# SunJiamei/LRP-ImageCaptioning

Measured on AMD Instinct MI355X. Metric: LRP heatmaps/sec (per predicted token) VGG16+adaptive-attn, 224x224, higher is better.
Workload: dtype bf16x3; 1 GPU; batch=32 synthetic 224x224 per GPU, VGG16 + adaptive-attention, LRP per-token heat-maps, 10 words/caption, V=10000 (BASELINE configs[1]); parallelism=image-sharded x1, RCCL weight broadcast, reverse_walk_precision=bf16x3, handles_per_gpu=2

## Files before the change

### lrp-imagecaptioning_amd/csrc/common.h

```cpp
#pragma once
#include <hip/hip_runtime.h>
#include <atomic>
#include <cstdarg>
#include <cstdio>
#include <cstdlib>
#include <string>
#include <vector>

#include "../../include/lrp_hip.h"

namespace lrp {

inline std::atomic<unsigned long long> g_launch_count{0};
#undef hipLaunchKernelGGL
#define hipLaunchKernelGGL(kernelName, numBlocks, numThreads, memPerBlock, streamId, ...)                  \
  do {                                                                                                    \
    ::lrp::g_launch_count.fetch_add(1, std::memory_order_relaxed);                                       \
    kernelName<<<(numBlocks), (numThreads), (memPerBlock), (streamId)>>>(__VA_ARGS__);                   \
  } while (0)

std::string& last_error_ref();

struct Switches {
  int conv_halo = 1;
  int conv_breg = 1;
  int conv_breg8 = 1;
  int conv_breg4 = 1;
  int conv_small = 1;
  int conv_mid = 1;
  int epi_fast = 1;
  int up2_pw = 1;
  int tile_order = 1;
  int fwd_emit = 1;
  int fwd_il = 1;
  int img_fused = 1;
  int up2_compact = 1;
  int img_fold = 1;
  int pool_fused = 1;
  int sparse_pool = 1;
  void load() {
    *this = Switches();
    auto rd = [](const char* name, int& v) { if (const char* e = getenv(name)) v = atoi(e); };
    rd("LRP_CONV_HALO", conv_halo); rd("LRP_CONV_BREG", conv_breg); rd("LRP_CONV_SMALL", conv_small);
    rd("LRP_CONV_MID", conv_mid); rd("LRP_EPI_FAST", epi_fast); rd("LRP_UP2_PW", up2_pw); rd("LRP_TILE_ORDER", tile_order);
    rd("LRP_FWD_EMIT", fwd_emit); rd("LRP_FWD_IL", fwd_il); rd("LRP_IMG_FUSED", img_fused); rd("LRP_UP2_COMPACT", up2_compact);
    rd("LRP_IMG_FOLD", img_fold); rd("LRP_SPARSE_POOL", sparse_pool); rd("LRP_POOL_FUSED", pool_fused);
    if (const char* e = getenv("LRP_CONV_BREG8")) conv_breg8 = atoi(e);
    if (const char* e = getenv("LRP_CONV_BREG4")) conv_breg4 = atoi(e);
  }
};
inline Switches& sw() {
  static Switches s = [] { Switches t; t.load(); return t; }();
  return s;
}

inline int fail(int code, const char* fmt, ...) {
  char buf[512];
  va_list ap;
  va_start(ap, fmt);
  vsnprintf(buf, sizeof(buf), fmt, ap);
  va_end(ap);
  last_error_ref() = buf;
  return code;
}

#define LRP_HIP_CHECK(expr)                                                                     \
  do {                                                                                          \
    hipError_t _e = (expr);                                                                     \
    if (_e != hipSuccess)                                                                       \
      return ::lrp::fail(LRP_ERR_HIP, "%s failed: %s (%s:%d)", #expr, hipGetErrorString(_e), \
                         __FILE__, __LINE__);                                                   \
  } while (0)

#define LRP_TRY(expr)         \
  do {                        \
    int _rc = (expr);         \
    if (_rc != LRP_OK) return _rc; \
  } while (0)

struct DevBuf {
  void* p = nullptr;
  size_t bytes = 0;
  bool owned = true;
  DevBuf() = default;
  DevBuf(const DevBuf&) = delete;
  DevBuf& operator=(const DevBuf&) = delete;
  DevBuf(DevBuf&& o) noexcept : p(o.p), bytes(o.bytes), owned(o.owned) { o.p = nullptr; o.bytes = 0; o.owned = true; }
  DevBuf& operator=(DevBuf&& o) noexcept {
    if (this != &o) { release(); p = o.p; bytes = o.bytes; owned = o.owned; o.p = nullptr; o.bytes = 0; o.owned = true; }
    return *this;
  }
  ~DevBuf() { release(); }
  void release() {
    if (p && owned) (void)hipFree(p);
    p = nullptr;
    bytes = 0;
    owned = true;
  }
  void view_of(const DevBuf& arena, size_t offset, size_t n) {
    release();
    p = static_cast<char*>(arena.p) + offset;
    bytes = n;
    owned = false;
  }
  int alloc(size_t n, int64_t* total) {
    release();
    if (n == 0) n = 16;
    hipError_t e = hipMalloc(&p, n);
    if (e != hipSuccess) {
      p = nullptr;
      (void)hipGetLastError();
      return fail(LRP_ERR_NOMEM, "device memory: hipMalloc(%zu bytes) failed: %s", n, hipGetErrorString(e));
    }
    bytes = n;
    if (total) *total += (int64_t)n;
    return LRP_OK;
  }
  template <typename T>
  T* as() const { return reinterpret_cast<T*>(p); }
};

struct ProfileRec {
  hipEvent_t e0, e1;
  double flop;
};
struct Profiler {
  bool on = false;
  ProfileRec cur{};
  std::vector<ProfileRec> recs;
  void begin(hipStream_t st) {
    if (on) { (void)hipEventCreate(&cur.e0); (void)hipEventCreate(&cur.e1); (void)hipEventRecord(cur.e0, st); }
  }
  void end(hipStream_t st, double flop) {
    if (on) { (void)hipEventRecord(cur.e1, st); cur.flop = flop; recs.push_back(cur); }
  }
  template <typename F>
  void drain(F each) {
    for (ProfileRec& p : recs) {
      float t = 0.f;
      if (hipEventSynchronize(p.e1) == hipSuccess && hipEventElapsedTime(&t, p.e0, p.e1) == hipSuccess) each((double)t, p.flop);
      (void)hipEventDestroy(p.e0); (void)hipEventDestroy(p.e1);
    }
    recs.clear();
  }
  int records(int cap, double* ms_out, double* flop_out, int* n_out) {
    int k = 0;
    drain([&](double ms, double flop) { if (k < cap) { ms_out[k] = ms; flop_out[k] = flop; ++k; } });
    *n_out = k;
    return LRP_OK;
  }
  int query(int64_t* launches, double* ms, double* flop) {
    int64_t nl = 0; double tm = 0, fl = 0;
    drain([&](double t, double f) { tm += t; fl += f; ++nl; });
    if (launches) *launches = nl;
    if (ms) *ms = tm;
    if (flop) *flop = fl;
    return LRP_OK;
  }
};

}
```

### lrp-imagecaptioning_amd/csrc/conv_sparse.h

```cpp
#pragma once
#include "cnn_kernels.h"
#include "conv_igemm.h"

namespace lrp {

typedef __bf16 bf16x16 __attribute__((ext_vector_type(16)));
typedef unsigned u32x2 __attribute__((ext_vector_type(2)));

struct SparseArgs {
  const float* sc;
  const unsigned* idxp;
  const float* wsp;
  const float* gate;
  float* out;
  const int* row2img;
  int NB, Hp, Wp, C, N;
  int cols_t, m_tiles, n_tiles;
  int out_plain;
  int diag;
};

constexpr int SP_TW = 14, SP_PITCH = SP_TW + 2;
constexpr int SP_BPACK = 32768, SP_NSTAGE = 4;

template <int WMW_, int WNW_, int MI_, int NJ_, int TH_>
struct SparseTile {
  static constexpr int WMW = WMW_, WNW = WNW_, MI = MI_, NJ = NJ_, TH = TH_;
  static constexpr int NW = WMW * WNW, NT = 64 * NW;
  static constexpr int BM = WMW * MI * 32, BN = WNW * NJ * 32;
  static constexpr int NENT = (TH + 2) * SP_PITCH;
  static constexpr int PENT = NENT + 1;
  static constexpr int SUB = PENT * 16;
  static constexpr int ABUF = 3 * SUB;
  static constexpr int SUBPIECES = (PENT + 63) / 64;
  static constexpr int APIECES = 3 * SUBPIECES;
  static constexpr int ASLOTS = (APIECES + NW - 1) / NW;
  static constexpr int PLANE = BN * 16;
  static constexpr int BSTAGE = 8 * PLANE;
  static constexpr int BPIECES = BSTAGE / 1024 / NW;
  static constexpr int NSLAB = BM / 64;
  static constexpr int EPI_P = 64 * (BN / 8) / NT;
  static constexpr int LDS = SP_NSTAGE * BSTAGE + 2 * ABUF + 128;
  static_assert(TH * SP_TW <= BM && BM % 64 == 0 && 256 % BN == 0, "tile");
  static_assert(BPIECES * NW * 1024 == BSTAGE && EPI_P * NT == 64 * (BN / 8), "pieces");
  static_assert(SP_NSTAGE * BSTAGE >= 64 * BN * 4, "the epilogue's C slab lies in the B stages");
  static_assert((TH + 2) * 4 <= 128, "image table");
  static_assert(LDS <= 160 * 1024, "LDS");
  static_assert(PENT >= 64, "a DMA piece is 64 windows");
};
typedef SparseTile<2, 4, 4, 2, 18> SparseTileLarge;
typedef SparseTile<2, 2, 1, 2, 4> SparseTileSmall;

__host__ __device__ inline int sparse_slot_tap(int q, int group, int slot) {
  const int qy = q >> 1, qx = q & 1, sy = qy ? 1 : -1, sx = qx ? 1 : -1;
  int dy, dx;
  if (group == 0) { dy = (slot >> 1) - qy; dx = (slot & 1) - qx; }
  else if (group == 1) {
    if (slot < 2) { dy = slot - qy; dx = sx; }
    else if (slot == 2) { dy = sy; dx = sx; }
    else return -1;
  } else {
    if (slot < 2) { dy = sy; dx = slot - qx; }
    else return -1;
  }
  return 3 * (dy + 1) + (dx + 1);
}

__global__ __launch_bounds__(256) void conv_sparse_index_kernel(const unsigned char* __restrict__ pos, unsigned* __restrict__ idxp, size_t n_sets,
                                                                int HW, int C) {
  for (size_t i = (size_t)blockIdx.x * 256 + threadIdx.x; i < n_sets * 4; i += (size_t)gridDim.x * 256) {
    const int q = (int)(i & 3);
    const size_t set = i >> 2;
    const u32x2 pp = *reinterpret_cast<const u32x2*>(pos + set * 8);
    const unsigned qxm = (q & 1) ? 0x01010101u : 0u, qym = (q >> 1) ? 0x01010101u : 0u;
    unsigned word[4][2];
#pragma unroll
    for (int d = 0; d < 2; ++d) {
      const unsigned P = pp[d];
      const unsigned px = P & 0x01010101u, py = (P >> 1) & 0x01010101u;
      const unsigned mh = px ^ qxm, mv = py ^ qym;
      const unsigned nmh = mh ^ 0x01010101u, nmv = mv ^ 0x01010101u;
      word[0][d] = P | ((P ^ 0x01010101u) << 2);
      word[1][d] = py | nmh | (nmh << 1);
      word[2][d] = (0x02020202u | ((mh & mv) ^ 0x01010101u)) << 2;
      word[3][d] = (px & mv) | (nmv << 1) | 0x0C0C0C0Cu;
    }
    unsigned h0[4], h1[4];
#pragma unroll
    for (int pl = 0; pl < 4; ++pl) {
      const unsigned t0 = word[pl][0] | (word[pl][0] >> 4), t1 = word[pl][1] | (word[pl][1] >> 4);
      h0[pl] = (t0 & 0xFFu) | (((t0 >> 16) & 0xFFu) << 8);
      h1[pl] = (t1 & 0xFFu) | (((t1 >> 16) & 0xFFu) << 8);
    }
    const u32x4 iw = {h0[0] | (h0[1] << 16), h0[2] | (h0[3] << 16), h1[0] | (h1[1] << 16), h1[2] | (h1[3] << 16)};
    const int spw = C >> 3;
    const size_t win = set / spw;
    const int sw = (int)(set - win * spw), chunk = sw >> 1, s2 = sw & 1;
    const size_t img = win / HW, pix = win - img * HW;
    reinterpret_cast<u32x4*>(idxp)[((((img * 4 + q) * (C >> 4) + chunk) * HW + pix) << 1) + s2] = iw;
  }
}

__global__ __launch_bounds__(256) void conv_sparse_pairs_kernel(const float* __restrict__ sc, float* __restrict__ scp, size_t n_sets, int HW, int C) {
  for (size_t i = (size_t)blockIdx.x * 256 + threadIdx.x; i < n_sets; i += (size_t)gridDim.x * 256) {
    float v[8];
    *reinterpret_cast<f32x4*>(v) = *reinterpret_cast<const f32x4*>(sc + i * 8);
    *reinterpret_cast<f32x4*>(v + 4) = *reinterpret_cast<const f32x4*>(sc + i * 8 + 4);
    const int spw = C >> 3;
    const size_t win = i / spw;
    const int sw = (int)(i - win * spw), chunk = sw >> 1, s2 = sw & 1;
    const size_t n = win / HW, pix = win - n * HW;
    split8_store(v, scp + ((((n * (C >> 4) + chunk) * HW + pix) << 1) + s2) * 8);
  }
}

__global__ __launch_bounds__(256) void conv_sparse_relayout_kernel(const float* __restrict__ pairs, float* __restrict__ scp, size_t n_sets, int HW, int C) {
  for (size_t i = (size_t)blockIdx.x * 256 + threadIdx.x; i < n_sets; i += (size_t)gridDim.x * 256) {
    const u32x4 hi = *reinterpret_cast<const u32x4*>(pairs + i * 8), lo = *reinterpret_cast<const u32x4*>(pairs + i * 8 + 4);
    const int spw = C >> 3;
    const size_t win = i / spw;
    const int sw_ = (int)(i - win * spw), chunk = sw_ >> 1, s2 = sw_ & 1;
    const size_t n = win / HW, pix = win - n * HW;
    float* dst = scp + ((((n * (C >> 4) + chunk) * HW + pix) << 1) + s2) * 8;
    *reinterpret_cast<u32x4*>(dst) = hi;
    *reinterpret_cast<u32x4*>(dst + 4) = lo;
  }
}

__global__ __launch_bounds__(256) void conv_sparse_pack_kernel(const float* __restrict__ wb, float* __restrict__ wsp, int N, int C, int CPo,
                                                               int n_tiles) {
  const size_t total = (size_t)4 * n_tiles * (C / 16) * 6 * 2 * 2 * 256;
  for (size_t i = (size_t)blockIdx.x * 256 + threadIdx.x; i < total; i += (size_t)gridDim.x * 256) {
    const int col = (int)(i & 255);
    size_t r = i >> 8;
    const int part = (int)(r & 1); r >>= 1;
    const int half = (int)(r & 1); r >>= 1;
    const int step = (int)(r % 6); r /= 6;
    const int chunk = (int)(r % (C / 16)); r /= (C / 16);
    const int nt = (int)(r % n_tiles);
    const int q = (int)(r / n_tiles);
    const int ci = nt * 256 + col;
    bf16x8 hi, lo;
#pragma unroll
    for (int e = 0; e < 8; ++e) {
      const int k32 = 16 * half + 8 * part + e, cb = k32 >> 2, slot = k32 & 3;
      const int ch8 = 4 * ((cb >> 1) & 1) + 2 * (cb >> 2) + (cb & 1);
      const int co = chunk * 16 + (step & 1) * 8 + ch8;
      const int tap = sparse_slot_tap(q, step >> 1, slot);
      const float v = (tap >= 0 && ci < N && co < C) ? wb[(size_t)ci * 9 * CPo + (size_t)tap * CPo + co] : 0.f;
      hi[e] = (__bf16)v;
      lo[e] = (__bf16)(v - (float)hi[e]);
    }
    const size_t sbase = ((((size_t)q * n_tiles + nt) * (C / 16) + chunk) * 6 + step) * (SP_BPACK / 16);
    u32x4* dst = reinterpret_cast<u32x4*>(wsp);
    dst[sbase + ((0 * 2 + half) * 2 + part) * 256 + col] = __builtin_bit_cast(u32x4, hi);
    dst[sbase + ((1 * 2 + half) * 2 + part) * 256 + col] = __builtin_bit_cast(u32x4, lo);
  }
}

template <class TL>
__global__ __launch_bounds__(TL::NT, 2) void conv_sparse_kernel(SparseArgs a) {
#if defined(__HIP_DEVICE_COMPILE__)
  constexpr int MI = TL::MI, NJ = TL::NJ, NW = TL::NW, NT = TL::NT, BN = TL::BN, TH = TL::TH;
  constexpr int NENT = TL::NENT, PENT = TL::PENT, SUB = TL::SUB, ABUF = TL::ABUF, BSTAGE = TL::BSTAGE, PLANE = TL::PLANE;
  __shared__ __attribute__((aligned(16))) unsigned char lds[TL::LDS];
  const int tid = threadIdx.x, lane = tid & 63, wave = tid >> 6, wm = wave / TL::WNW, wn = wave % TL::WNW;
  const int l31 = lane & 31, half = lane >> 5;
  const int per_class = a.m_tiles * a.n_tiles;
  const int q = blockIdx.x / per_class, rem = blockIdx.x - q * per_class;
  const int nt = rem / a.m_tiles, mt = rem - nt * a.m_tiles;
  const int qy = q >> 1, qx = q & 1, sy = qy ? 1 : -1, sx = qx ? 1 : -1;
  const int tyt = mt / a.cols_t, txt = mt - tyt * a.cols_t;
  const int Y0 = tyt * TH, x0 = txt * SP_TW;
  const int Hp = a.Hp, Wp = a.Wp, C = a.C, N = a.N, H = 2 * Hp, W = 2 * Wp;
  const int nys = a.NB * Hp;
  const int n0 = nt * BN;
  const int nt256 = n0 >> 8, ncol0 = n0 & 255;
  const float inv_Hp = 1.0f / (float)Hp;
  auto divmod = [](int x, int d, float inv, int& qq, int& r) {
    qq = (int)(((float)x + 0.5f) * inv);
    r = x - qq * d;
    if (r < 0) { --qq; r += d; } else if (r >= d) { ++qq; r -= d; }
  };
  unsigned char* Bs = lds;
  unsigned char* As = lds + SP_NSTAGE * BSTAGE;

  auto chunk0 = [&](int e) { return e * 16 + half * 8; };
  int e_own[MI], e_h[MI], e_v[MI], e_d[MI];
#pragma unroll
  for (int i = 0; i < MI; ++i) {
    const int r = (wm * MI + i) * 32 + l31;
    const int ty = r / SP_TW, tx = r - ty * SP_TW;
    const int Ys = Y0 + ty, wx = x0 + tx;
    int n_, wy;
    divmod(Ys, Hp, inv_Hp, n_, wy);
    const bool ok = r < TH * SP_TW && Ys < nys && wx < Wp;
    const bool okh = ok && wx + sx >= 0 && wx + sx < Wp, okv = ok && wy + sy >= 0 && wy + sy < Hp;
    const int e = (ty + 1) * SP_PITCH + tx + 1;
    e_own[i] = chunk0(ok ? e : NENT);
    e_h[i] = chunk0(okh ? e + sx : NENT);
    e_v[i] = chunk0(okv ? e + sy * SP_PITCH : NENT);
    e_d[i] = chunk0(okh && okv ? e + sy * SP_PITCH + sx : NENT);
  }

  typedef __attribute__((address_space(3))) void* lptr_t;
  constexpr int RSRC_FLAGS = 0x00020000;
  const int nchunks = C >> 4, nsteps = nchunks * 6;
  const __amdgpu_buffer_rsrc_t rsB = __builtin_amdgcn_make_buffer_rsrc(
      (void*)(reinterpret_cast<const unsigned char*>(a.wsp) + ((size_t)q * (N >> 8) + nt256) * (size_t)nsteps * SP_BPACK), 0, nsteps * SP_BPACK, RSRC_FLAGS);
  const int wave_s = __builtin_amdgcn_readfirstlane(wave);
  auto fire_b = [&](int step, int stage) {
#pragma unroll
    for (int p = 0; p < TL::BPIECES; ++p) {
      const int pc = wave_s * TL::BPIECES + p;
      const int plane = pc / (BN / 64), sub = pc - plane * (BN / 64);
      __builtin_amdgcn_raw_ptr_buffer_load_lds(rsB, (lptr_t)(Bs + stage * BSTAGE + pc * 1024), 16, lane * 16,
                                               step * SP_BPACK + plane * 4096 + (ncol0 + sub * 64) * 16, 0, 0);
    }
  };

  int* imgtab = reinterpret_cast<int*>(As + 2 * ABUF);
  if (tid < TH + 2) {
    const int Ys = Y0 - 1 + tid;
    int n_, wy;
    divmod(Ys >= 0 && Ys < nys ? Ys : 0, Hp, inv_Hp, n_, wy);
    imgtab[tid] = a.row2img ? a.row2img[n_] : n_;
  }
  const __amdgpu_buffer_rsrc_t rsS = __builtin_amdgcn_make_buffer_rsrc((void*)a.sc, 0, 0x7FFFFFFF, RSRC_FLAGS);
  const __amdgpu_buffer_rsrc_t rsI = __builtin_amdgcn_make_buffer_rsrc((void*)a.idxp, 0, 0x7FFFFFFF, RSRC_FLAGS);
  constexpr int OOB = (int)0x80000000;
  auto fire_a = [&](int slot, int set8, int abuf) {
    int wv = wave_s, ln = lane;
    asm volatile("" : "+s"(wv), "+v"(ln));
    int pj = wv + NW * slot;
    if (pj >= TL::APIECES) pj = TL::APIECES - 1;
    const int pl = pj / TL::SUBPIECES, jp = pj - pl * TL::SUBPIECES;
    const int first = jp * 64 < PENT - 64 ? jp * 64 : PENT - 64;
    const int e = first + ln;
    const int hy = e >> 4, hx = e & 15;
    const int Ys = Y0 - 1 + hy, wx = x0 - 1 + hx;
    const bool ok = e < NENT && Ys >= 0 && Ys < nys && wx >= 0 && wx < Wp;
    int n_, wy;
    divmod(ok ? Ys : 0, Hp, inv_Hp, n_, wy);
    const int chunk = set8 >> 1, s = set8 & 1;
    int vo;
    if (pl < 2) {
      vo = ((((n_ * (C >> 4) + chunk) * Hp + wy) * Wp + wx) << 6) + s * 32 + pl * 16;
    } else {
      const int img = imgtab[ok ? hy : 0];
      vo = (((((img * 4 + q) * (C >> 4) + chunk) * Hp + wy) * Wp + wx) << 5) + s * 16;
    }
    __builtin_amdgcn_raw_ptr_buffer_load_lds(pl < 2 ? rsS : rsI, (lptr_t)(As + abuf * ABUF + pl * SUB + first * 16), 16, ok ? vo : OOB,
                                             0, 0, 0);
  };
  auto fire_set = [&](int set8, int abuf) {
#pragma unroll
    for (int sl = 0; sl < TL::ASLOTS; ++sl) fire_a(sl, set8, abuf);
  };

  const int nsteps2 = nchunks * 6;
  auto bsrc = [&](int chunk, int t6) { return chunk * 6 + 2 * (t6 % 3) + t6 / 3; };
  __syncthreads();
  fire_set(0, 0);
  if (nchunks * 2 > 1) fire_set(1, 1);
  fire_b(bsrc(0, 0), 0);
  fire_b(bsrc(0, 1), 1);
  asm volatile("s_waitcnt vmcnt(0)" ::: "memory");
  __syncthreads();

  f32x16 acc[MI][NJ];
#pragma unroll
  for (int i = 0; i < MI; ++i)
#pragma unroll
    for (int j = 0; j < NJ; ++j)
#pragma unroll
      for (int r = 0; r < 16; ++r) acc[i][j][r] = 0.f;

  const int bcol = (wn * (NJ * 32) + l31) * 16 + half * (2 * PLANE);
  auto expand = [](u32x2 x) -> bf16x8 {
    const u32x4 r = {x[0] & 0xFFFFu, x[0] >> 16, x[1] & 0xFFFFu, x[1] >> 16};
    return __builtin_bit_cast(bf16x8, r);
  };
  auto pairup = [](u32x2 h, u32x2 d) -> bf16x8 {
    const u32x4 r = {__builtin_amdgcn_perm(d[0], h[0], 0x05040100u), __builtin_amdgcn_perm(d[0], h[0], 0x07060302u),
                     __builtin_amdgcn_perm(d[1], h[1], 0x05040100u), __builtin_amdgcn_perm(d[1], h[1], 0x07060302u)};
    return __builtin_bit_cast(bf16x8, r);
  };
  auto ld8 = [](const unsigned char* p) { return *reinterpret_cast<const u32x2*>(p); };
  auto ld2 = [](const unsigned char* p) { return (unsigned)*reinterpret_cast<const unsigned short*>(p); };
  struct BF { bf16x16 h[NJ], l[NJ]; };
  auto load_b = [&](BF& b, const unsigned char* Bb) {
#pragma unroll
    for (int j = 0; j < NJ; ++j) {
      const unsigned char* bp = Bb + j * 512;
      const bf16x8 h0 = *reinterpret_cast<const bf16x8*>(bp), h1 = *reinterpret_cast<const bf16x8*>(bp + PLANE);
      const bf16x8 l0 = *reinterpret_cast<const bf16x8*>(bp + 4 * PLANE), l1 = *reinterpret_cast<const bf16x8*>(bp + 4 * PLANE + PLANE);
      b.h[j] = __builtin_shufflevector(h0, h1, 0, 1, 2, 3, 4, 5, 6, 7, 8, 9, 10, 11, 12, 13, 14, 15);
      b.l[j] = __builtin_shufflevector(l0, l1, 0, 1, 2, 3, 4, 5, 6, 7, 8, 9, 10, 11, 12, 13, 14, 15);
    }
  };
  auto kstep = [&](const unsigned char* Ab, int grp, const BF& b) {
    const unsigned char* Ah = Ab;
    const unsigned char* Al = Ab + SUB;
    const unsigned char* Ai = Ab + 2 * SUB;
#pragma unroll
    for (int i = 0; i < MI; ++i) {
      bf16x8 vh, vl;
      int ix;
      if (grp == 1) {
        const int oh = e_h[i], od = e_d[i];
        vh = pairup(ld8(Ah + oh), ld8(Ah + od));
        vl = pairup(ld8(Al + oh), ld8(Al + od));
        ix = (int)(ld2(Ai + oh + 2) | ld2(Ai + od + 4));
      } else {
        const int oo = grp == 0 ? e_own[i] : e_v[i];
        vh = expand(ld8(Ah + oo));
        vl = expand(ld8(Al + oo));
        ix = (int)ld2(Ai + oo + (grp == 0 ? 0 : 6));
      }
#pragma unroll
      for (int j = 0; j < NJ; ++j) {
        acc[i][j] = __builtin_amdgcn_smfmac_f32_32x32x32_bf16(vl, b.h[j], acc[i][j], ix, 0, 0);
        acc[i][j] = __builtin_amdgcn_smfmac_f32_32x32x32_bf16(vh, b.l[j], acc[i][j], ix, 0, 0);
        acc[i][j] = __builtin_amdgcn_smfmac_f32_32x32x32_bf16(vh, b.h[j], acc[i][j], ix, 0, 0);
      }
    }
  };

  for (int chunk = 0; chunk < nchunks; ++chunk) {
    const bool next_chunk = chunk + 1 < nchunks;
#pragma unroll
    for (int ss = 0; ss < 3; ++ss) {
      const int t0 = 2 * ss, t1 = 2 * ss + 1;
      const int st0 = chunk * 6 + t0;
      if (st0 + 2 < nsteps2) {
        const int nc = ss == 2 ? chunk + 1 : chunk, nt0 = (t0 + 2) % 6;
        fire_b(bsrc(nc, nt0), (st0 + 2) & 3);
        fire_b(bsrc(nc, nt0 + 1), (st0 + 3) & 3);
      }
      if (ss == 2 && next_chunk) fire_set(2 * chunk + 2, 0);
      if (ss == 0 && chunk > 0) fire_set(2 * chunk + 1, 1);
      BF b0, b1;
      load_b(b0, Bs + (st0 & 3) * BSTAGE + bcol);
      load_b(b1, Bs + ((st0 + 1) & 3) * BSTAGE + bcol);
      kstep(As + (t0 / 3) * ABUF, t0 % 3, b0);
      kstep(As + (t1 / 3) * ABUF, t1 % 3, b1);
      asm volatile("s_waitcnt vmcnt(0) lgkmcnt(0)\n\ts_barrier" ::: "memory");
    }
  }

  float* Cs = reinterpret_cast<float*>(lds);
#pragma unroll
  for (int sl = 0; sl < TL::NSLAB; ++sl) {
    f32x4 g[TL::EPI_P][2];
    bool ok4[TL::EPI_P];
    size_t off4[TL::EPI_P];
#pragma unroll
    for (int p = 0; p < TL::EPI_P; ++p) {
      const int item = tid + p * NT, row = item / (BN / 8), cg = item % (BN / 8);
      const int R = sl * 64 + row;
      const int ty = R / SP_TW, tx = R - ty * SP_TW;
      const int Ys = Y0 + ty, wx = x0 + tx;
      int n_, wy;
      divmod(Ys < nys ? Ys : 0, Hp, inv_Hp, n_, wy);
      const int col = n0 + cg * 8;
      ok4[p] = R < TH * SP_TW && Ys < nys && wx < Wp && col < N && !((a.diag & 1) && (row | cg | sl));
      const int y = 2 * wy + qy, x = 2 * (wx < Wp ? wx : 0) + qx;
      const int img = a.row2img ? a.row2img[n_] : n_;
      const size_t goff = (((size_t)img * H + y) * W + x) * N + (col < N ? col : 0);
      off4[p] = (((size_t)n_ * H + y) * W + x) * N + (col < N ? col : 0);
      g[p][0] = *reinterpret_cast<const f32x4*>(a.gate + goff);
      g[p][1] = *reinterpret_cast<const f32x4*>(a.gate + goff + 4);
    }
    if (sl) __syncthreads();
    float* cw = Cs + (4 * half) * BN + wn * (NJ * 32) + l31;
#pragma unroll
    for (int ii = 0; ii < 2; ++ii) {
      const int f = 2 * sl + ii;
      if (wm == f / MI) {
#pragma unroll
        for (int r = 0; r < 16; ++r)
#pragma unroll
          for (int j = 0; j < NJ; ++j) cw[(ii * 32 + (r & 3) + 8 * (r >> 2)) * BN + j * 32] = acc[f % MI][j][r];
      }
    }
    __syncthreads();
#pragma unroll
    for (int p = 0; p < TL::EPI_P; ++p) {
      if (!ok4[p]) continue;
      const int item = tid + p * NT, row = item / (BN / 8), cg = item % (BN / 8);
      const f32x4 c0 = *reinterpret_cast<const f32x4*>(Cs + row * BN + cg * 8), c1 = *reinterpret_cast<const f32x4*>(Cs + row * BN + cg * 8 + 4);
      float r[8];
#pragma unroll
      for (int e = 0; e < 4; ++e) { r[e] = c0[e] * g[p][0][e]; r[4 + e] = c1[e] * g[p][1][e]; }
      float* dst = a.out + off4[p];
      if (a.out_plain) {
        *reinterpret_cast<f32x4*>(dst) = *reinterpret_cast<const f32x4*>(r);
        *reinterpret_cast<f32x4*>(dst + 4) = *reinterpret_cast<const f32x4*>(r + 4);
      } else {
        split8_store(r, dst);
      }
    }
  }
#endif
}

inline size_t conv_sparse_weight_floats(int N, int C) { return (size_t)4 * ((N + 255) / 256) * (C / 16) * 6 * (SP_BPACK / 4); }
inline bool conv_sparse_supports(int N, int C, int Hp, int Wp) { return N % 256 == 0 && C % 16 == 0 && Hp >= 1 && Wp >= 1; }

inline hipError_t conv_sparse_pack(const float* wb_dev, float* wsp_dev, int N, int C, hipStream_t st) {
  const int n_tiles = (N + 255) / 256;
  const size_t total = (size_t)4 * n_tiles * (C / 16) * 6 * 2 * 2 * 256;
  hipLaunchKernelGGL(conv_sparse_pack_kernel, dim3((unsigned)((total + 255) / 256)), dim3(256), 0, st, wb_dev, wsp_dev, N, C, conv_cinp(C), n_tiles);
  return hipGetLastError();
}

inline size_t conv_sparse_index_words(int images, int Hp, int Wp, int C) { return (size_t)images * Hp * Wp * (C / 8) * 4 * 4; }
inline hipError_t conv_sparse_index(const unsigned char* pos_dev, unsigned* idxp_dev, int images, int Hp, int Wp, int C, hipStream_t st) {
  const size_t n_sets = (size_t)images * Hp * Wp * (C / 8);
  hipLaunchKernelGGL(conv_sparse_index_kernel, dim3(stream_grid(n_sets * 4)), dim3(256), 0, st, pos_dev, idxp_dev, n_sets, Hp * Wp, C);
  return hipGetLastError();
}
inline hipError_t conv_sparse_pairs(const float* sc_dev, float* scp_dev, int NB, int Hp, int Wp, int C, hipStream_t st) {
  const size_t n_sets = (size_t)NB * Hp * Wp * (C / 8);
  hipLaunchKernelGGL(conv_sparse_pairs_kernel, dim3(stream_grid(n_sets)), dim3(256), 0, st, sc_dev, scp_dev, n_sets, Hp * Wp, C);
  return hipGetLastError();
}

constexpr long CONV_SPARSE_SMALL_BLOCKS = 96L;
inline long conv_sparse_large_blocks(int NB, int Hp, int Wp, int N) {
  return 4L * ((NB * Hp + SparseTileLarge::TH - 1) / SparseTileLarge::TH) * ((Wp + SP_TW - 1) / SP_TW) * (N / SparseTileLarge::BN);
}
inline bool conv_sparse_small_grid(int NB, int Hp, int Wp, int N) {
  return sw().conv_small != 0 && conv_sparse_large_blocks(NB, Hp, Wp, N) <= CONV_SPARSE_SMALL_BLOCKS;
}

template <class TL>
inline hipError_t conv_sparse_launch_tile(SparseArgs a, hipStream_t st) {
  a.cols_t = (a.Wp + SP_TW - 1) / SP_TW;
  a.n_tiles = a.N / TL::BN;
  a.m_tiles = ((a.NB * a.Hp + TL::TH - 1) / TL::TH) * a.cols_t;
  hipLaunchKernelGGL(conv_sparse_kernel<TL>, dim3(4 * a.m_tiles * a.n_tiles), dim3(TL::NT), 0, st, a);
  return hipGetLastError();
}

inline hipError_t conv_sparse_launch(SparseArgs a, hipStream_t st) {
  if (!conv_sparse_supports(a.N, a.C, a.Hp, a.Wp) || !a.sc || !a.idxp || !a.wsp || !a.gate || !a.out) return hipErrorInvalidValue;
  if (a.NB <= 0) return hipSuccess;
  const bool small = (a.diag & 4) ? true : (a.diag & 2) ? false : conv_sparse_small_grid(a.NB, a.Hp, a.Wp, a.N);
  return small ? conv_sparse_launch_tile<SparseTileSmall>(a, st) : conv_sparse_launch_tile<SparseTileLarge>(a, st);
}

}
```

Measured before the change: 10960 heatmaps/s.

## Stream sparse-conv B fragments into registers and double-buffer A chunks in LDS

Adds a WREG variant of the large-tile sparse conv kernel. Weight (B) fragments now go from global memory straight into a three-deep register ring instead of through four LDS stages, and the A windows for a whole chunk are double-buffered in LDS. A reads for the next step are software-pipelined between the MFMA calls, and the block syncs once per chunk instead of after every step pair. This frees LDS and removes per-step barriers, at the cost of more VGPR pressure and redundant per-wave global B loads. It is on by default for the large tile and includes an A/B profiling script.

Result: faster. 11120 heatmaps/s, median of 6 (+1.5%).

```diff
diff --git a/lrp-imagecaptioning_amd/csrc/common.h b/lrp-imagecaptioning_amd/csrc/common.h
--- a/lrp-imagecaptioning_amd/csrc/common.h
+++ b/lrp-imagecaptioning_amd/csrc/common.h
@@ -26,6 +26,7 @@
   int conv_breg = 1;
   int conv_breg8 = 1;
   int conv_breg4 = 1;
+  int conv_sparse_wreg = 1;
   int conv_small = 1;
   int conv_mid = 1;
   int epi_fast = 1;
@@ -47,6 +48,7 @@
     rd("LRP_IMG_FOLD", img_fold); rd("LRP_SPARSE_POOL", sparse_pool); rd("LRP_POOL_FUSED", pool_fused);
     if (const char* e = getenv("LRP_CONV_BREG8")) conv_breg8 = atoi(e);
     if (const char* e = getenv("LRP_CONV_BREG4")) conv_breg4 = atoi(e);
+    if (const char* e = getenv("LRP_CONV_SPARSE_WREG")) conv_sparse_wreg = atoi(e);
   }
 };
 inline Switches& sw() {
diff --git a/lrp-imagecaptioning_amd/csrc/conv_sparse.h b/lrp-imagecaptioning_amd/csrc/conv_sparse.h
--- a/lrp-imagecaptioning_amd/csrc/conv_sparse.h
+++ b/lrp-imagecaptioning_amd/csrc/conv_sparse.h
@@ -41,11 +41,16 @@
   static constexpr int NSLAB = BM / 64;
   static constexpr int EPI_P = 64 * (BN / 8) / NT;
   static constexpr int LDS = SP_NSTAGE * BSTAGE + 2 * ABUF + 128;
+  static constexpr int CBUF = 2 * ABUF;
+  static constexpr int CSLOTS = 6;
+  static constexpr int LDS_WREG = 2 * CBUF + 128 > 64 * BN * 4 ? 2 * CBUF + 128 : 64 * BN * 4;
   static_assert(TH * SP_TW <= BM && BM % 64 == 0 && 256 % BN == 0, "tile");
   static_assert(BPIECES * NW * 1024 == BSTAGE && EPI_P * NT == 64 * (BN / 8), "pieces");
   static_assert(SP_NSTAGE * BSTAGE >= 64 * BN * 4, "the epilogue's C slab lies in the B stages");
   static_assert((TH + 2) * 4 <= 128, "image table");
   static_assert(LDS <= 160 * 1024, "LDS");
+  static_assert(2 * CBUF <= 65536, "WREG: every A address is an immediate offset of a ds_read");
+  static_assert(SUBPIECES <= NW, "WREG: a wave moves one piece of every sub-plane");
   static_assert(PENT >= 64, "a DMA piece is 64 windows");
 };
 typedef SparseTile<2, 4, 4, 2, 18> SparseTileLarge;
@@ -158,12 +163,13 @@
   }
 }
 
-template <class TL>
+template <class TL, bool WREG>
 __global__ __launch_bounds__(TL::NT, 2) void conv_sparse_kernel(SparseArgs a) {
 #if defined(__HIP_DEVICE_COMPILE__)
   constexpr int MI = TL::MI, NJ = TL::NJ, NW = TL::NW, NT = TL::NT, BN = TL::BN, TH = TL::TH;
   constexpr int NENT = TL::NENT, PENT = TL::PENT, SUB = TL::SUB, ABUF = TL::ABUF, BSTAGE = TL::BSTAGE, PLANE = TL::PLANE;
-  __shared__ __attribute__((aligned(16))) unsigned char lds[TL::LDS];
+  constexpr int CBUF = TL::CBUF;
+  __shared__ __attribute__((aligned(16))) unsigned char lds[WREG ? TL::LDS_WREG : TL::LDS];
   const int tid = threadIdx.x, lane = tid & 63, wave = tid >> 6, wm = wave / TL::WNW, wn = wave % TL::WNW;
   const int l31 = lane & 31, half = lane >> 5;
   const int per_class = a.m_tiles * a.n_tiles;
@@ -176,14 +182,19 @@
   const int nys = a.NB * Hp;
   const int n0 = nt * BN;
   const int nt256 = n0 >> 8, ncol0 = n0 & 255;
-  const float inv_Hp = 1.0f / (float)Hp;
+  float inv_Hp = 1.0f / (float)Hp;
+  if constexpr (WREG) {
+    float sc_;
+    asm volatile("v_readfirstlane_b32 %0, %1" : "=s"(sc_) : "v"(inv_Hp));
+    inv_Hp = sc_;
+  }
   auto divmod = [](int x, int d, float inv, int& qq, int& r) {
     qq = (int)(((float)x + 0.5f) * inv);
     r = x - qq * d;
     if (r < 0) { --qq; r += d; } else if (r >= d) { ++qq; r -= d; }
   };
-  unsigned char* Bs = lds;
-  unsigned char* As = lds + SP_NSTAGE * BSTAGE;
+  [[maybe_unused]] unsigned char* Bs = lds;
+  unsigned char* As = WREG ? lds : lds + SP_NSTAGE * BSTAGE;
 
   auto chunk0 = [&](int e) { return e * 16 + half * 8; };
   int e_own[MI], e_h[MI], e_v[MI], e_d[MI];
@@ -219,7 +230,7 @@
     }
   };
 
-  int* imgtab = reinterpret_cast<int*>(As + 2 * ABUF);
+  int* imgtab = reinterpret_cast<int*>(As + (WREG ? 2 * CBUF : 2 * ABUF));
   if (tid < TH + 2) {
     const int Ys = Y0 - 1 + tid;
     int n_, wy;
@@ -229,17 +240,12 @@
   const __amdgpu_buffer_rsrc_t rsS = __builtin_amdgcn_make_buffer_rsrc((void*)a.sc, 0, 0x7FFFFFFF, RSRC_FLAGS);
   const __amdgpu_buffer_rsrc_t rsI = __builtin_amdgcn_make_buffer_rsrc((void*)a.idxp, 0, 0x7FFFFFFF, RSRC_FLAGS);
   constexpr int OOB = (int)0x80000000;
-  auto fire_a = [&](int slot, int set8, int abuf) {
-    int wv = wave_s, ln = lane;
-    asm volatile("" : "+s"(wv), "+v"(ln));
-    int pj = wv + NW * slot;
-    if (pj >= TL::APIECES) pj = TL::APIECES - 1;
-    const int pl = pj / TL::SUBPIECES, jp = pj - pl * TL::SUBPIECES;
+  auto fire_piece = [&](int pl, int jp, int ln, int set8, unsigned char* dst, bool live) {
     const int first = jp * 64 < PENT - 64 ? jp * 64 : PENT - 64;
     const int e = first + ln;
     const int hy = e >> 4, hx = e & 15;
     const int Ys = Y0 - 1 + hy, wx = x0 - 1 + hx;
-    const bool ok = e < NENT && Ys >= 0 && Ys < nys && wx >= 0 && wx < Wp;
+    const bool ok = live && e < NENT && Ys >= 0 && Ys < nys && wx >= 0 && wx < Wp;
     int n_, wy;
     divmod(ok ? Ys : 0, Hp, inv_Hp, n_, wy);
     const int chunk = set8 >> 1, s = set8 & 1;
@@ -250,8 +256,15 @@
       const int img = imgtab[ok ? hy : 0];
       vo = (((((img * 4 + q) * (C >> 4) + chunk) * Hp + wy) * Wp + wx) << 5) + s * 16;
     }
-    __builtin_amdgcn_raw_ptr_buffer_load_lds(pl < 2 ? rsS : rsI, (lptr_t)(As + abuf * ABUF + pl * SUB + first * 16), 16, ok ? vo : OOB,
-                                             0, 0, 0);
+    __builtin_amdgcn_raw_ptr_buffer_load_lds(pl < 2 ? rsS : rsI, (lptr_t)(dst + pl * SUB + first * 16), 16, ok ? vo : OOB, 0, 0, 0);
+  };
+  auto fire_a = [&](int slot, int set8, int abuf) {
+    int wv = wave_s, ln = lane;
+    asm volatile("" : "+s"(wv), "+v"(ln));
+    int pj = wv + NW * slot;
+    if (pj >= TL::APIECES) pj = TL::APIECES - 1;
+    const int pl = pj / TL::SUBPIECES;
+    fire_piece(pl, pj - pl * TL::SUBPIECES, ln, set8, As + abuf * ABUF, true);
   };
   auto fire_set = [&](int set8, int abuf) {
 #pragma unroll
@@ -260,11 +273,24 @@
 
   const int nsteps2 = nchunks * 6;
   auto bsrc = [&](int chunk, int t6) { return chunk * 6 + 2 * (t6 % 3) + t6 / 3; };
+  auto fire_chunk_piece = [&](int slot, int chunk, int cbuf, bool live) {
+    int wv = wave_s;
+    asm volatile("" : "+s"(wv));
+    int ln;
+    asm volatile("v_mbcnt_lo_u32_b32 %0, -1, 0\n\tv_mbcnt_hi_u32_b32 %0, -1, %0" : "=&v"(ln));
+    const int s2 = slot / 3;
+    fire_piece(slot % 3, wv < TL::SUBPIECES ? wv : TL::SUBPIECES - 1, ln, 2 * chunk + s2, As + cbuf * CBUF + s2 * ABUF, live);
+  };
   __syncthreads();
-  fire_set(0, 0);
-  if (nchunks * 2 > 1) fire_set(1, 1);
-  fire_b(bsrc(0, 0), 0);
-  fire_b(bsrc(0, 1), 1);
+  if constexpr (WREG) {
+#pragma unroll
+    for (int sl = 0; sl < TL::CSLOTS; ++sl) fire_chunk_piece(sl, 0, 0, true);
+  } else {
+    fire_set(0, 0);
+    if (nchunks * 2 > 1) fire_set(1, 1);
+    fire_b(bsrc(0, 0), 0);
+    fire_b(bsrc(0, 1), 1);
+  }
   asm volatile("s_waitcnt vmcnt(0)" ::: "memory");
   __syncthreads();
 
@@ -299,31 +325,133 @@
       b.l[j] = __builtin_shufflevector(l0, l1, 0, 1, 2, 3, 4, 5, 6, 7, 8, 9, 10, 11, 12, 13, 14, 15);
     }
   };
-  auto kstep = [&](const unsigned char* Ab, int grp, const BF& b) {
+  [[maybe_unused]] int e_oh[MI], e_vd[MI];
+  if constexpr (WREG) {
+    static_assert(PENT * 16 < 65536, "offsets fit 16 bits");
+#pragma unroll
+    for (int i = 0; i < MI; ++i) { e_oh[i] = e_own[i] | (e_h[i] << 16); e_vd[i] = e_v[i] | (e_d[i] << 16); }
+  }
+  auto eoff = [&](int i, int which) -> int {
+    if constexpr (WREG) {
+      int o;
+      const int pk = which < 2 ? e_oh[i] : e_vd[i];
+      if (which & 1) asm volatile("v_lshrrev_b32 %0, 16, %1" : "=v"(o) : "v"(pk));
+      else asm volatile("v_and_b32 %0, 0xffff, %1" : "=v"(o) : "v"(pk));
+      return o;
+    } else {
+      return which == 0 ? e_own[i] : which == 1 ? e_h[i] : which == 2 ? e_v[i] : e_d[i];
+    }
+  };
+  struct AF { bf16x8 vh, vl; int ix; };
+  struct AR { u32x2 h0, h1, l0, l1; unsigned i0, i1; };
+  auto read_raw = [&](int i, const unsigned char* Ab, int grp) -> AR {
     const unsigned char* Ah = Ab;
     const unsigned char* Al = Ab + SUB;
     const unsigned char* Ai = Ab + 2 * SUB;
+    AR r{};
+    if (grp == 1) {
+      const int oh = eoff(i, 1), od = eoff(i, 3);
+      r.h0 = ld8(Ah + oh); r.h1 = ld8(Ah + od);
+      r.l0 = ld8(Al + oh); r.l1 = ld8(Al + od);
+      r.i0 = ld2(Ai + oh + 2); r.i1 = ld2(Ai + od + 4);
+    } else {
+      const int oo = eoff(i, grp == 0 ? 0 : 2);
+      r.h0 = ld8(Ah + oo);
+      r.l0 = ld8(Al + oo);
+      r.i0 = ld2(Ai + oo + (grp == 0 ? 0 : 6));
+    }
+    return r;
+  };
+  auto finish_a = [&](const AR& r, int grp) -> AF {
+    AF f;
+    if (grp == 1) {
+      f.vh = pairup(r.h0, r.h1);
+      f.vl = pairup(r.l0, r.l1);
+      f.ix = (int)(r.i0 | r.i1);
+    } else {
+      f.vh = expand(r.h0);
+      f.vl = expand(r.l0);
+      f.ix = (int)r.i0;
+    }
+    return f;
+  };
+  auto read_a = [&](int i, const unsigned char* Ab, int grp) -> AF { return finish_a(read_raw(i, Ab, grp), grp); };
+  auto mma3 = [&](f32x16& c, const AF& f, bf16x16 bh, bf16x16 bl) {
+    c = __builtin_amdgcn_smfmac_f32_32x32x32_bf16(f.vl, bh, c, f.ix, 0, 0);
+    c = __builtin_amdgcn_smfmac_f32_32x32x32_bf16(f.vh, bl, c, f.ix, 0, 0);
+    c = __builtin_amdgcn_smfmac_f32_32x32x32_bf16(f.vh, bh, c, f.ix, 0, 0);
+  };
+
+  if constexpr (WREG) {
+    struct BW { u32x4 h[2], l[2]; };
+    BW bq[3];
+    static_assert(NJ == 2, "two column fragments per step: a chunk is twelve, a multiple of the ring");
+    const int bvo = (ncol0 + wn * (NJ * 32) + l31) * 16 + half * (2 * 4096);
+    auto load_bw = [&](BW& b, int chunk, int f) {
+      int st = bsrc(chunk + f / 12, (f % 12) >> 1);
+      st = st < nsteps2 ? st : nsteps2 - 1;
+      const int so = st * SP_BPACK, vo = bvo + (f & 1) * 512;
+#pragma unroll
+      for (int part = 0; part < 2; ++part) {
+        b.h[part] = __builtin_amdgcn_raw_buffer_load_b128(rsB, vo, so + part * 4096, 0);
+        b.l[part] = __builtin_amdgcn_raw_buffer_load_b128(rsB, vo, so + (4 + part) * 4096, 0);
+      }
+    };
+    auto whole = [](u32x4 p0, u32x4 p1) -> bf16x16 {
+      return __builtin_shufflevector(__builtin_bit_cast(bf16x8, p0), __builtin_bit_cast(bf16x8, p1), 0, 1, 2, 3, 4, 5, 6, 7, 8, 9, 10, 11, 12,
+                                     13, 14, 15);
+    };
+#pragma unroll
+    for (int f = 0; f < 3; ++f) load_bw(bq[f], 0, f);
+    AF aq[MI];
+    AR raw;
+#pragma unroll
+    for (int i = 0; i < MI; ++i) aq[i] = read_a(i, As, 0);
+    for (int chunk = 0; chunk < nchunks; ++chunk) {
+      const unsigned char* Ac = As + (chunk & 1) * CBUF;
+      const unsigned char* An = As + ((chunk & 1) ^ 1) * CBUF;
+      const bool next_chunk = chunk + 1 < nchunks;
+#pragma unroll
+      for (int s = 0; s < 6; ++s) {
+        if (s == 5) {
+          asm volatile("s_waitcnt vmcnt(16) lgkmcnt(0)\n\ts_barrier" ::: "memory");
+        }
+        const int ns = (s + 1) % 6;
+        const unsigned char* Ax = (s == 5 ? An : Ac) + (ns / 3) * ABUF;
+        __builtin_amdgcn_sched_barrier(0);
+#pragma unroll
+        for (int j = 0; j < NJ; ++j) {
+          const int f = 2 * s + j;
+          BW& b = bq[f % 3];
+          const bf16x16 bh = whole(b.h[0], b.h[1]), bl = whole(b.l[0], b.l[1]);
+#pragma unroll
+          for (int i = 0; i < MI; ++i) {
+            mma3(acc[i][j], aq[i], bh, bl);
+            if (j == NJ - 1) {
+              if (i > 0) aq[i - 1] = finish_a(raw, ns % 3);
+              raw = read_raw(i, Ax, ns % 3);
+              __builtin_amdgcn_sched_barrier(0);
+            }
+          }
+          __builtin_amdgcn_sched_barrier(0);
+          if (j == 0 && s < 4) {
+#pragma unroll
+            for (int sl = s; sl < TL::CSLOTS; sl += 4) fire_chunk_piece(sl, chunk + 1, (chunk & 1) ^ 1, next_chunk);
+          }
+          load_bw(b, chunk, f + 3);
+          __builtin_amdgcn_sched_barrier(0);
+        }
+        aq[MI - 1] = finish_a(raw, ns % 3);
+      }
+    }
+    __syncthreads();
+  } else {
+  auto kstep = [&](const unsigned char* Ab, int grp, const BF& b) {
 #pragma unroll
     for (int i = 0; i < MI; ++i) {
-      bf16x8 vh, vl;
-      int ix;
-      if (grp == 1) {
-        const int oh = e_h[i], od = e_d[i];
-        vh = pairup(ld8(Ah + oh), ld8(Ah + od));
-        vl = pairup(ld8(Al + oh), ld8(Al + od));
-        ix = (int)(ld2(Ai + oh + 2) | ld2(Ai + od + 4));
-      } else {
-        const int oo = grp == 0 ? e_own[i] : e_v[i];
-        vh = expand(ld8(Ah + oo));
-        vl = expand(ld8(Al + oo));
-        ix = (int)ld2(Ai + oo + (grp == 0 ? 0 : 6));
-      }
-#pragma unroll
-      for (int j = 0; j < NJ; ++j) {
-        acc[i][j] = __builtin_amdgcn_smfmac_f32_32x32x32_bf16(vl, b.h[j], acc[i][j], ix, 0, 0);
-        acc[i][j] = __builtin_amdgcn_smfmac_f32_32x32x32_bf16(vh, b.l[j], acc[i][j], ix, 0, 0);
-        acc[i][j] = __builtin_amdgcn_smfmac_f32_32x32x32_bf16(vh, b.h[j], acc[i][j], ix, 0, 0);
-      }
+      const AF f = read_a(i, Ab, grp);
+#pragma unroll
+      for (int j = 0; j < NJ; ++j) mma3(acc[i][j], f, b.h[j], b.l[j]);
     }
   };
 
@@ -348,6 +476,7 @@
       asm volatile("s_waitcnt vmcnt(0) lgkmcnt(0)\n\ts_barrier" ::: "memory");
     }
   }
+  }
 
   float* Cs = reinterpret_cast<float*>(lds);
 #pragma unroll
@@ -435,12 +564,12 @@
   return sw().conv_small != 0 && conv_sparse_large_blocks(NB, Hp, Wp, N) <= CONV_SPARSE_SMALL_BLOCKS;
 }
 
-template <class TL>
+template <class TL, bool WREG>
 inline hipError_t conv_sparse_launch_tile(SparseArgs a, hipStream_t st) {
   a.cols_t = (a.Wp + SP_TW - 1) / SP_TW;
   a.n_tiles = a.N / TL::BN;
   a.m_tiles = ((a.NB * a.Hp + TL::TH - 1) / TL::TH) * a.cols_t;
-  hipLaunchKernelGGL(conv_sparse_kernel<TL>, dim3(4 * a.m_tiles * a.n_tiles), dim3(TL::NT), 0, st, a);
+  hipLaunchKernelGGL((conv_sparse_kernel<TL, WREG>), dim3(4 * a.m_tiles * a.n_tiles), dim3(TL::NT), 0, st, a);
   return hipGetLastError();
 }
 
@@ -448,7 +577,8 @@
   if (!conv_sparse_supports(a.N, a.C, a.Hp, a.Wp) || !a.sc || !a.idxp || !a.wsp || !a.gate || !a.out) return hipErrorInvalidValue;
   if (a.NB <= 0) return hipSuccess;
   const bool small = (a.diag & 4) ? true : (a.diag & 2) ? false : conv_sparse_small_grid(a.NB, a.Hp, a.Wp, a.N);
-  return small ? conv_sparse_launch_tile<SparseTileSmall>(a, st) : conv_sparse_launch_tile<SparseTileLarge>(a, st);
-}
-
-}
+  if (small) return conv_sparse_launch_tile<SparseTileSmall, false>(a, st);
+  return sw().conv_sparse_wreg ? conv_sparse_launch_tile<SparseTileLarge, true>(a, st) : conv_sparse_launch_tile<SparseTileLarge, false>(a, st);
+}
+
+}
diff --git a/profiles/sparse_wreg_ab.py b/profiles/sparse_wreg_ab.py
--- /dev/null
+++ b/profiles/sparse_wreg_ab.py
@@ -0,0 +1,56 @@
+#!/usr/bin/env python3
+import os, sys, statistics
+import numpy as np
+sys.path.insert(0, os.path.dirname(os.path.dirname(os.path.abspath(__file__))))
+PASSES = int(sys.argv[1]) if len(sys.argv) > 1 else 5
+import torch
+from bench import synth_weights
+from lrp_imagecaptioning_amd.engine import LRPEngine, switches
+from lrp_imagecaptioning_amd.synthetic import VGG16_CFG, captions, images
+B, T, V = 32, 10, 10000
+eng = LRPEngine(decoder="adaptive", V=V, max_images=B, max_tokens=B * T, max_caption_len=T + 1)
+eng.set_weights(synth_weights(0, V))
+rs = np.random.RandomState(1)
+X = torch.as_tensor(images(rs, B)).cuda()
+caps = captions(rs, B, T, V)
+idx = [b for b in range(B) for _ in range(T)]
+tpos = [t for _ in range(B) for t in range(1, T + 1)]
+out = torch.empty((B * T, 224, 224, 3), dtype=torch.float32, device="cuda")
+eng.encode_images(X); eng.decoder_forward(caps)
+ref = {}
+for on in (1, 0):
+    with switches(LRP_CONV_SPARSE_WREG=on):
+        eng.explain_tokens(idx, tpos, out=out); torch.cuda.synchronize()
+        ref[on] = out.clone()
+print("heat-maps bit-identical on/off:", bool(torch.equal(ref[0], ref[1])), "finite:", bool(torch.isfinite(ref[1]).all()),
+      "non-zero:", float(ref[1].abs().sum()) > 0, flush=True)
+del ref
+
+names = [c[0] for c in VGG16_CFG][::-1]
+res = {0: [], 1: []}
+for p in range(PASSES):
+    for on in (0, 1):
+        with switches(LRP_CONV_SPARSE_WREG=on):
+            eng.explain_tokens(idx, tpos, out=out); torch.cuda.synchronize()
+            eng.profile_enable(True)
+            acc = None
+            for _ in range(3):
+                eng.explain_tokens(idx, tpos, out=out); torch.cuda.synchronize()
+                rec = eng.profile_records()
+                acc = rec if acc is None else [(a + b, f) for (a, f), (b, _) in zip(acc, rec)]
+            eng.profile_enable(False)
+            res[on].append([m / 3 for m, _ in acc])
+        print("pass %d WREG=%d walk %.3f ms: %s" % (p, on, sum(res[on][-1]), " ".join("%.3f" % m for m in res[on][-1])), flush=True)
+print("records per walk:", len(res[0][0]), names[:len(res[0][0])])
+print("%-14s %28s %28s" % ("class", "WREG=0 med [min,max]", "WREG=1 med [min,max]"))
+
+
+def line(name, v0, v1):
+    won = statistics.median(v1) < min(v0)
+    print("%-14s %28s %28s %s" % (name, "%.3f [%.3f, %.3f]" % (statistics.median(v0), min(v0), max(v0)),
+                                  "%.3f [%.3f, %.3f]" % (statistics.median(v1), min(v1), max(v1)), "WON" if won else ""))
+
+
+for k in range(len(res[0][0])):
+    line(names[k] if k < len(names) else str(k), [r[k] for r in res[0]], [r[k] for r in res[1]])
+line("walk total", [sum(r) for r in res[0]], [sum(r) for r in res[1]])
```
